# skyhehe123/SA-SSD

Measured on NVIDIA H100. Metric: KITTI frames/sec (~20k pts, car_cfg voxel grid), higher is better.
Workload: dtype f32

## Files before the change

sa-ssd_b200/csrc/spconv_split.cu:

```cuda
#include "tc_common.cuh"

namespace sps {

using namespace tc;

constexpr int BKC = 64;
constexpr int PROD_WARPS = 8;
constexpr int THREADS3 = CONS_THREADS + PROD_WARPS * 32;
constexpr int W_PROD = CONS_THREADS / 32;
constexpr int CLUSTER = 2;
constexpr int SPLIT_TILES_MAX = 74;

template <int BN>
struct Cfg3 {
    static constexpr int B_TILE_BYTES = BN * 128;
    static constexpr int STAGE_BYTES = 2 * A_TILE_BYTES + 2 * B_TILE_BYTES;
    static constexpr int STAGES = 4;
    static constexpr int NBR_TILE_BYTES = BM * 27 * 4;
    static constexpr int SMEM_BYTES = STAGES * STAGE_BYTES + 2 * NBR_TILE_BYTES + 1024 + 512 + 256;
};

__device__ __forceinline__ void cp_async16(uint32_t dst, const void* src, uint32_t src_bytes) {
    asm volatile("cp.async.cg.shared.global [%0], [%1], 16, %2;" ::"r"(dst), "l"(src), "r"(src_bytes) : "memory");
}
__device__ __forceinline__ void st_shared_zero16(uint32_t dst) {
    asm volatile("st.shared.v4.b32 [%0], {%1, %1, %1, %1};" ::"r"(dst), "r"(0u) : "memory");
}
__device__ __forceinline__ void cp_async_arrive_noinc(uint32_t bar) {
    asm volatile("cp.async.mbarrier.arrive.noinc.shared::cta.b64 [%0];" ::"r"(bar) : "memory");
}
__device__ __forceinline__ void mbar_arrive_remote(uint32_t bar, uint32_t rank) {
    asm volatile(
        "{\n\t"
        ".reg .b32 ra;\n\t"
        "mapa.shared::cluster.u32 ra, %0, %1;\n\t"
        "mbarrier.arrive.release.cluster.shared::cluster.b64 _, [ra];\n\t"
        "}\n" ::"r"(bar), "r"(rank) : "memory");
}
__device__ __forceinline__ void mbar_wait_cluster(uint32_t bar, uint32_t parity) {
    asm volatile(
        "{\n\t"
        ".reg .pred p;\n\t"
        "WAITC_LOOP:\n\t"
        "mbarrier.try_wait.parity.acquire.cluster.shared::cta.b64 p, [%0], %1;\n\t"
        "@p bra.uni WAITC_DONE;\n\t"
        "bra.uni WAITC_LOOP;\n\t"
        "WAITC_DONE:\n\t"
        "}\n" ::"r"(bar), "r"(parity) : "memory");
}

struct Args {
    const __half* in;
    size_t in_plane;
    const void* wpack;
    const float* scale;
    const float* shift;
    const int* nbr;
    const int* tile_mask;
    const int* d_rows;
    __half* out_split;
    size_t out_plane;
    float* out_f32;
    float* scratch;
    int* counters;
    int cin, cout, taps, rows_cap, relu, out_ch, out_f32_stride;
};

struct ChunkSet {
    uint32_t mask;
    __device__ __forceinline__ ChunkSet(uint32_t tap_mask, int tpg, int nchunks, int part, int nparts) {
        uint32_t act = tap_mask;
        if (tpg > 1) {
            const uint32_t group = (1u << tpg) - 1u;
            act = 0u;
            for (int g = 0; g < nchunks; ++g)
                if ((tap_mask >> (g * tpg)) & group) act |= 1u << g;
        }
        if (nparts == 1) { mask = act; return; }
        uint32_t m = 0u, rest = act;
        for (int j = 0; rest; ++j) {
            const uint32_t low = rest & (0u - rest);
            if ((j & 1) == part) m |= low;
            rest ^= low;
        }
        mask = m;
    }
};

template <int TABLE, int BN>
__global__ void __cluster_dims__(CLUSTER, 1, 1) __launch_bounds__(THREADS3, 1) spconv_split_kernel(const Args p) {
    using C = Cfg3<BN>;
    extern __shared__ uint8_t smem_raw[];
    const uint32_t base = (smem_u32(smem_raw) + 1023u) & ~1023u;
    uint8_t* base_ptr = smem_raw + (base - smem_u32(smem_raw));
    const uint32_t nbr_base = base + C::STAGES * C::STAGE_BYTES;
    const int* nbr_smem = (const int*)(base_ptr + C::STAGES * C::STAGE_BYTES);
    const uint32_t bar_base = nbr_base + 2 * C::NBR_TILE_BYTES;
    auto full_a = [&](int s, int w) { return bar_base + 512u + 8u * (s * PROD_WARPS + w); };
    auto full_b = [&](int s) { return bar_base + 8u * (C::STAGES + s); };
    auto empty = [&](int s) { return bar_base + 8u * (3 * C::STAGES + s); };
    auto nbr_full = [&](int b) { return bar_base + 8u * (4 * C::STAGES + 4 + b); };
    auto nbr_empty = [&](int b) { return bar_base + 8u * (4 * C::STAGES + 6 + b); };
    const uint32_t peer_done = bar_base + 8u * (4 * C::STAGES + 8);

    pdl_launch_dependents();
    const int warp = __shfl_sync(0xffffffffu, (int)(threadIdx.x >> 5), 0), lane = threadIdx.x & 31;
    const int cin = p.cin;
    const int ppt = cin >> 3;
    const int tpg = (BKC % cin == 0) ? BKC / cin : 1;
    const int nchunks = (p.taps + tpg - 1) / tpg;
    const bool nbr_tiles = TABLE && p.taps <= 27;
    const uint32_t all_taps = p.taps >= 32 ? 0xffffffffu : ((1u << p.taps) - 1u);

    if (threadIdx.x == 0) {
        for (int s = 0; s < C::STAGES; ++s) {
            for (int w = 0; w < PROD_WARPS; ++w) mbar_init(full_a(s, w), 32);
            mbar_init(full_b(s), 1);
            mbar_init(empty(s), 2);
        }
        for (int b = 0; b < 2; ++b) { mbar_init(nbr_full(b), 1); mbar_init(nbr_empty(b), PROD_WARPS); }
        mbar_init(peer_done, 128);
        fence_barrier_init();
    }
    __syncthreads();
    cluster_sync_all();
    pdl_wait();
    const int M = p.d_rows ? min(__ldg(p.d_rows), p.rows_cap) : p.rows_cap;
    const int ntiles = (M + BM - 1) / BM;
    const uint32_t crank = cluster_ctarank();
    const int G = (int)gridDim.x;
    const int R = ntiles / G, rem = ntiles - R * G;
    const bool tail_split = TABLE && p.scratch && nchunks > 1 && R == 0 && rem > 0 && 2 * rem <= G &&
                            rem <= SPLIT_TILES_MAX;
    const int n_items = R + ((tail_split ? (int)(blockIdx.x >> 1) < rem : (int)blockIdx.x < rem) ? 1 : 0);
    struct Item { int tile, part, nparts; };
    auto item_at = [&](int i) {
        Item it;
        if (i < R) { it.tile = (int)blockIdx.x + i * G; it.part = 0; it.nparts = 1; }
        else if (tail_split) { it.tile = R * G + (int)(blockIdx.x >> 1); it.part = (int)crank; it.nparts = 2; }
        else { it.tile = R * G + (int)blockIdx.x; it.part = 0; it.nparts = 1; }
        return it;
    };
    auto chunks_of = [&](const Item& it) {
        uint32_t tm = all_taps;
        if (TABLE && p.tile_mask) {
            tm = (uint32_t)__ldg(&p.tile_mask[it.tile]) & all_taps;
            if (!tm) tm = 1u;
        }
        return ChunkSet(tm, tpg, nchunks, it.part, it.nparts).mask;
    };
    auto rot_of = [&](int tile) { return (int)(((unsigned)tile * 11u) % (unsigned)nchunks); };

    if (warp >= W_PROD) {
        const int pw = warp - W_PROD;
        const bool loader = pw == 0 && lane == 0;
        const int piece = lane & 7, oct = lane >> 3;
        const int tl = piece / ppt, pc8 = (piece - tl * ppt) * 8;
        uint32_t offs[4];
        int rowt[4];
#pragma unroll
        for (int j = 0; j < 4; ++j) {
            const int r = pw * 16 + j * 4 + oct;
            offs[j] = (uint32_t)(r >> 3) * 1024u + (uint32_t)(r & 7) * 128u + (((uint32_t)piece ^ (uint32_t)(r & 7)) << 4);
            rowt[j] = r * p.taps;
        }
        const __half* in_hi = p.in + pc8;
        const __half* in_lo = in_hi + p.in_plane;
        int stage = 0;
        uint32_t phase = 0;
        int nb = 0;
        uint32_t nb_phase = 0;
        int ld_nb = 0;
        uint32_t ld_nb_phase = 0;
        auto load_nbr = [&](int tile) {
            const int rows_here = min(BM, p.rows_cap - tile * BM);
            const uint32_t bytes = (uint32_t)(rows_here * p.taps * 4) & ~15u;
            mbar_wait(nbr_empty(ld_nb), ld_nb_phase ^ 1u);
            mbar_expect_tx(nbr_full(ld_nb), bytes);
            if (bytes) bulk_g2s(nbr_base + ld_nb * C::NBR_TILE_BYTES, p.nbr + (size_t)tile * BM * p.taps, bytes, nbr_full(ld_nb));
            if (++ld_nb == 2) { ld_nb = 0; ld_nb_phase ^= 1u; }
        };
        if (loader && nbr_tiles && n_items > 0) load_nbr(item_at(0).tile);
        for (int ii = 0; ii < n_items; ++ii) {
            const Item item = item_at(ii);
            const int tile = item.tile;
            const int rows_here = min(BM, p.rows_cap - tile * BM);
            const int rows_copied = nbr_tiles ? ((rows_here * p.taps * 4) & ~15) / (p.taps * 4) : 0;
            const int* ntile = nbr_smem + nb * (C::NBR_TILE_BYTES / 4);
            const uint32_t cmask = chunks_of(item);
            const int m0 = tile * BM + pw * 16 + oct;
            if (nbr_tiles) {
                if (lane == 0) mbar_wait(nbr_full(nb), nb_phase);
                __syncwarp();
            }
            const int rot = rot_of(tile);
            auto chunk_at = [&](int gi) { return gi + rot < nchunks ? gi + rot : gi + rot - nchunks; };
            auto next_active = [&](int gi) {
                for (++gi; gi < nchunks; ++gi)
                    if ((cmask >> chunk_at(gi)) & 1u) break;
                return gi;
            };
            auto load_srcs = [&](int g, int (&dst)[4]) {
                const int t = g * tpg + tl;
                const bool tap_ok = tl < tpg && t < p.taps;
#pragma unroll
                for (int j = 0; j < 4; ++j) {
                    const int m = m0 + 4 * j;
                    dst[j] = -1;
                    if (tap_ok && m < M)
                        dst[j] = TABLE ? ((nbr_tiles && pw * 16 + j * 4 + oct < rows_copied) ? ntile[rowt[j] + t]
                                                                                          : __ldg(&p.nbr[(size_t)m * p.taps + t])) : m;
                }
            };
            int gi = next_active(-1);
            int srcs[4] = {-1, -1, -1, -1};
            if (gi < nchunks) load_srcs(chunk_at(gi), srcs);
            while (gi < nchunks) {
                const int gi_next = next_active(gi);
                if (lane == 0) {
                    mbar_wait(empty(stage), phase ^ 1u);
                    if (loader) {
                        const uint32_t dst = base + stage * C::STAGE_BYTES + 2 * A_TILE_BYTES;
                        const uint8_t* src = (const uint8_t*)p.wpack + (size_t)chunk_at(gi) * (2 * C::B_TILE_BYTES);
                        mbar_expect_tx(full_b(stage), 2 * C::B_TILE_BYTES);
                        bulk_g2s(dst, src, 2 * C::B_TILE_BYTES, full_b(stage));
                    }
                }
                __syncwarp();
                int nxt[4] = {-1, -1, -1, -1};
                if (gi_next < nchunks) load_srcs(chunk_at(gi_next), nxt);
                const uint32_t a_hi = base + stage * C::STAGE_BYTES, a_lo = a_hi + A_TILE_BYTES;
#pragma unroll
                for (int j = 0; j < 4; ++j) {
                    const uint32_t nbytes = srcs[j] >= 0 ? 16u : 0u;
                    const uint32_t eo = (uint32_t)(srcs[j] < 0 ? 0 : srcs[j]) * (uint32_t)cin;
                    cp_async16(a_hi + offs[j], in_hi + eo, nbytes);
                    cp_async16(a_lo + offs[j], in_lo + eo, nbytes);
                }
                cp_async_arrive_noinc(full_a(stage, pw));
                if (++stage == C::STAGES) { stage = 0; phase ^= 1u; }
#pragma unroll
                for (int j = 0; j < 4; ++j) srcs[j] = nxt[j];
                gi = gi_next;
            }
            if (nbr_tiles) {
                __syncwarp();
                if (lane == 0) mbar_arrive(nbr_empty(nb));
                if (++nb == 2) { nb = 0; nb_phase ^= 1u; }
            }
            if (loader && nbr_tiles && ii + 1 < n_items) load_nbr(item_at(ii + 1).tile);
        }
    } else {
        const int wg = threadIdx.x >> 7, t = threadIdx.x & 127;
        float big[BN / 2], small[BN / 2];
        int stage = 0;
        uint32_t phase = 0;
        int executed = 0, tiles_done = 0;
        for (int ii = 0; ii < n_items; ++ii) {
            const Item item = item_at(ii);
            const int tile = item.tile, part = item.part;
            const bool split = item.nparts == 2;
            const uint32_t cmask = chunks_of(item);
#pragma unroll
            for (int i = 0; i < BN / 2; ++i) { big[i] = 0.f; small[i] = 0.f; }
            const int rot = rot_of(tile);
            int prev = -1;
            for (int ci = 0; ci < nchunks; ++ci) {
                const int ch = ci + rot < nchunks ? ci + rot : ci + rot - nchunks;
                if (!((cmask >> ch) & 1u)) continue;
#pragma unroll 1
                for (int w = 0; w < PROD_WARPS; ++w) mbar_wait(full_a(stage, w), phase);
                fence_proxy_async();
                mbar_wait(full_b(stage), phase);
                const uint32_t ah = base + stage * C::STAGE_BYTES + (uint32_t)wg * (A_TILE_BYTES / 2);
                const uint32_t bh = base + stage * C::STAGE_BYTES + 2 * A_TILE_BYTES;
                wgmma_fence();
                mma_chunk_x3<1, BN>(big, small, ah, ah + A_TILE_BYTES, bh, bh + C::B_TILE_BYTES);
                wgmma_commit();
                wgmma_wait<1>();
                if (prev >= 0 && t == 0) mbar_arrive(empty(prev));
                prev = stage;
                ++executed;
                if (++stage == C::STAGES) { stage = 0; phase ^= 1u; }
            }
            wgmma_wait<0>();
            fence_regs<BN / 2>(big);
            fence_regs<BN / 2>(small);
            if (prev >= 0 && t == 0) mbar_arrive(empty(prev));
            if (part == 0) ++tiles_done;
            const bool giver = split && wg != part;
            const int rl0 = wg * 64 + (t >> 5) * 16 + ((t & 31) >> 2);
            float* prow = split ? p.scratch + (size_t)(tile - R * G) * BM * BN : nullptr;
            if (split && !giver) {
                mbar_wait_cluster(peer_done, 0u);
            }
#pragma unroll
            for (int j = 0; j < BN / 8; ++j) {
                const int n = 8 * j + 2 * (t & 3);
                const float scl0 = (p.scale && n < p.cout) ? __ldg(&p.scale[n]) : 1.f;
                const float scl1 = (p.scale && n + 1 < p.cout) ? __ldg(&p.scale[n + 1]) : 1.f;
                const float shl0 = (p.shift && n < p.cout) ? __ldg(&p.shift[n]) : 0.f;
                const float shl1 = (p.shift && n + 1 < p.cout) ? __ldg(&p.shift[n + 1]) : 0.f;
#pragma unroll
                for (int i = 0; i < 2; ++i) {
                    const int rl = rl0 + 8 * i, m = tile * BM + rl;
                    float a0 = __fadd_rn(big[4 * j + 2 * i], small[4 * j + 2 * i] * (1.f / kF16LoScale));
                    float a1 = __fadd_rn(big[4 * j + 2 * i + 1], small[4 * j + 2 * i + 1] * (1.f / kF16LoScale));
                    float2* q = split ? (float2*)(prow + (size_t)rl * BN + n) : nullptr;
                    if (giver) {
                        *q = make_float2(a0, a1);
                        continue;
                    }
                    if (split) {
                        const float2 pq = __ldcg(q);
                        a0 = __fadd_rn(a0, pq.x);
                        a1 = __fadd_rn(a1, pq.y);
                    }
                    float o0 = fmaf(a0, scl0, shl0), o1 = fmaf(a1, scl1, shl1);
                    if (p.relu) { o0 = fmaxf(o0, 0.f); o1 = fmaxf(o1, 0.f); }
                    if (m < M) {
                        if (p.out_f32 && n < p.out_f32_stride)
                            *(float2*)(p.out_f32 + (size_t)m * p.out_f32_stride + n) = make_float2(o0, o1);
                        if (p.out_split && 8 * j < p.out_ch) {
                            uint32_t h, l;
                            split_f16x2(o0, o1, h, l);
                            __half* ohi = p.out_split + (size_t)m * p.out_ch + n;
                            *(uint32_t*)ohi = h;
                            *(uint32_t*)(ohi + p.out_plane) = l;
                        }
                    }
                }
            }
            if (giver) mbar_arrive_remote(peer_done, (uint32_t)(part ^ 1));
        }
        if (p.counters && threadIdx.x == 0 && executed) {
            atomicAdd(&p.counters[0], executed);
            atomicAdd(&p.counters[1], tiles_done);
        }
    }

    __syncthreads();
    cluster_sync_all();
}

template <int TABLE, int BN>
static int launch3(const Args& a, cudaStream_t stream) {
    using C = Cfg3<BN>;
    auto kern = spconv_split_kernel<TABLE, BN>;
    static int max_ctas = 0;
    if (!max_ctas) {
        if (cudaFuncSetAttribute(kern, cudaFuncAttributeMaxDynamicSharedMemorySize, C::SMEM_BYTES) != cudaSuccess)
            return SASSD_ERR_LAUNCH;
        cudaLaunchConfig_t cfg = {};
        cfg.gridDim = dim3(CLUSTER * sassd_div_up(sassd_num_sms(), CLUSTER)); cfg.blockDim = dim3(THREADS3);
        cfg.dynamicSmemBytes = C::SMEM_BYTES;
        int clusters = 0;
        if (cudaOccupancyMaxActiveClusters(&clusters, kern, &cfg) != cudaSuccess || clusters < 1) {
            cudaGetLastError();
            clusters = sassd_num_sms() / (2 * CLUSTER);
        }
        max_ctas = CLUSTER * (clusters < SPLIT_TILES_MAX ? clusters : SPLIT_TILES_MAX);
    }
    int grid = CLUSTER * sassd_div_up(a.rows_cap, BM);
    if (grid > max_ctas) grid = max_ctas;
    if (launch_pdl(kern, dim3(grid), dim3(THREADS3), C::SMEM_BYTES, stream, a) != cudaSuccess) return SASSD_ERR_LAUNCH;
    return sassd_check_launch();
}

template <int TABLE>
static int dispatch3(const Args& a, cudaStream_t s) {
    if (a.cout <= 16) return launch3<TABLE, 16>(a, s);
    if (a.cout <= 32) return launch3<TABLE, 32>(a, s);
    if (a.cout <= 64) return launch3<TABLE, 64>(a, s);
    return SASSD_ERR_UNSUPPORTED;
}

}

__global__ void spconv_pack_kernel(const float* __restrict__ w, int taps, int cin, int cs, int cout, int bn, int tpg,
                                   int nchunks, __half* __restrict__ out) {
    const long long per_chunk = 2LL * bn * 64;
    const long long total = (long long)nchunks * per_chunk;
    for (long long i = blockIdx.x * (long long)blockDim.x + threadIdx.x; i < total; i += (long long)gridDim.x * blockDim.x) {
        const int g = (int)(i / per_chunk);
        long long rem = i % per_chunk;
        const int part = (int)(rem / (bn * 64));
        rem %= (bn * 64);
        const int n = (int)(rem / 64), pos = (int)(rem % 64);
        const int kk = (((pos >> 3) ^ (n & 7)) << 3) + (pos & 7);
        const int tl = kk / cs, ch = kk % cs, t = g * tpg + tl;
        float v = 0.f;
        if (tl < tpg && t < taps && ch < cin && n < cout) v = w[((size_t)t * cin + ch) * cout + n];
        float hi, lo;
        tc::split_f16(v, hi, lo);
        out[i] = __float2half_rn(part == 0 ? hi : lo);
    }
}

static int spconv_bn(int cout) { return cout <= 16 ? 16 : (cout <= 32 ? 32 : 64); }
static int spconv_tpg(int cs) { return (64 % cs == 0) ? 64 / cs : 1; }

extern "C" size_t sassd_spconv_pack_bytes(int taps, int cin_stored, int cout) {
    if (taps < 1 || cin_stored < 8 || (cin_stored & 7) || cin_stored > 64 || cout < 1 || cout > 64) return 0;
    const int tpg = spconv_tpg(cin_stored);
    return (size_t)((taps + tpg - 1) / tpg) * 2 * spconv_bn(cout) * 128;
}

extern "C" int sassd_spconv_pack(const float* weight, int taps, int cin, int cin_stored, int cout, void* packed,
                                 sassd_stream_t stream_) {
    if (!weight || !packed || cin < 1 || cin > cin_stored || !sassd_spconv_pack_bytes(taps, cin_stored, cout))
        return SASSD_ERR_ARG;
    const int tpg = spconv_tpg(cin_stored), nchunks = (taps + tpg - 1) / tpg, bn = spconv_bn(cout);
    spconv_pack_kernel<<<sassd_grid((long long)nchunks * 2 * bn * 64, 256), 256, 0, (cudaStream_t)stream_>>>(
        weight, taps, cin, cin_stored, cout, bn, tpg, nchunks, (__half*)packed);
    return sassd_check_launch();
}

extern "C" size_t sassd_spconv_workspace_bytes(void) {
    return (size_t)sps::SPLIT_TILES_MAX * sps::BM * 64 * sizeof(float);
}

extern "C" int sassd_spconv_f16x3(const sassd_spconv_desc* d, const void* in_split, const void* wpack,
                                  const float* scale, const float* shift, const int32_t* nbr,
                                  const int32_t* tile_mask, const int32_t* d_rows, void* out_split, float* out_f32,
                                  void* ws, size_t ws_bytes, int32_t* counters, sassd_stream_t stream_) {
    if (!d || !in_split || !wpack || (!out_split && !out_f32)) return SASSD_ERR_ARG;
    if (d->cin < 8 || (d->cin & 7) || d->cin > 64 || d->cout < 1 || d->cout > 64 || d->taps < 1 || d->rows_cap < 0)
        return SASSD_ERR_ARG;
    if (d->taps > 1 && !nbr) return SASSD_ERR_ARG;
    if (tile_mask && d->taps > 27) return SASSD_ERR_ARG;
    if (out_split && ((d->out_ch & 7) || d->out_ch < d->cout)) return SASSD_ERR_ARG;
    if (out_f32 && (d->out_f32_stride & 3)) return SASSD_ERR_ARG;
    if (ws && ws_bytes < sassd_spconv_workspace_bytes()) return SASSD_ERR_WORKSPACE;
    if (d->rows_cap == 0) return SASSD_OK;
    sps::Args a;
    a.in = (const __half*)in_split; a.in_plane = (size_t)d->in_rows_cap * d->cin;
    a.wpack = wpack; a.scale = scale; a.shift = shift; a.nbr = nbr; a.tile_mask = tile_mask; a.d_rows = d_rows;
    a.out_split = (__half*)out_split; a.out_plane = (size_t)d->rows_cap * d->out_ch; a.out_f32 = out_f32;
    a.scratch = (float*)ws; a.counters = counters;
    a.cin = d->cin; a.cout = d->cout; a.taps = d->taps; a.rows_cap = d->rows_cap; a.relu = d->relu;
    a.out_ch = d->out_ch; a.out_f32_stride = d->out_f32_stride;
    return d->taps > 1 ? sps::dispatch3<1>(a, (cudaStream_t)stream_) : sps::dispatch3<0>(a, (cudaStream_t)stream_);
}

__global__ void features_to_split_kernel(const float* __restrict__ feat, const int* __restrict__ d_rows, int rows_cap,
                                         int cin, int cs, __half* __restrict__ out) {
    const int rows = d_rows ? min(*d_rows, rows_cap) : rows_cap;
    const long long total = (long long)rows * cs;
    const size_t plane = (size_t)rows_cap * cs;
    for (long long i = blockIdx.x * (long long)blockDim.x + threadIdx.x; i < total; i += (long long)gridDim.x * blockDim.x) {
        const int r = (int)(i / cs), c = (int)(i % cs);
        float hi = 0.f, lo = 0.f;
        if (c < cin) tc::split_f16(feat[(size_t)r * cin + c], hi, lo);
        out[i] = __float2half_rn(hi);
        out[i + plane] = __float2half_rn(lo);
    }
}

extern "C" int sassd_features_to_split(const float* feat, const int32_t* d_rows, int rows_cap, int cin, int cs,
                                       void* out_split, sassd_stream_t stream_) {
    if (!feat || !out_split || cin < 1 || cs < cin || (cs & 7)) return SASSD_ERR_ARG;
    if (rows_cap <= 0) return SASSD_OK;
    features_to_split_kernel<<<sassd_grid((long long)rows_cap * cs, 256), 256, 0, (cudaStream_t)stream_>>>(
        feat, d_rows, rows_cap, cin, cs, (__half*)out_split);
    return sassd_check_launch();
}

__global__ void split_rows_to_bev_kernel(const uint4* __restrict__ feat, size_t in_plane16, const int4* __restrict__ coors,
                                         const int* __restrict__ d_rows, int rows_cap, int C8, int D, int H, int W,
                                         size_t out_plane16, uint4* __restrict__ bev, int* __restrict__ tile_dist) {
    const int rows = min(*d_rows, rows_cap);
    const long long total = (long long)rows * C8;
    for (long long i = blockIdx.x * (long long)blockDim.x + threadIdx.x; i < total; i += (long long)gridDim.x * blockDim.x) {
        const int r = (int)(i / C8), q = (int)(i % C8);
        const int4 c = __ldg(&coors[r]);
        const size_t o = (((size_t)c.x * H + c.z) * W + c.w) * (size_t)(D * C8) + (size_t)c.y * C8 + q;
        bev[o] = __ldg(&feat[i]);
        bev[o + out_plane16] = __ldg(&feat[i + in_plane16]);
        if (tile_dist && q == 0) sassd_mark_conv2d_tiles(tile_dist, c.x, c.z, c.w, H, W);
    }
}

extern "C" int sassd_split_rows_to_bev(const void* feat_split, const int32_t* coors, const int32_t* d_rows, int rows_cap,
                                       int C, int D, int H, int W, int batch, void* bev_split, int32_t* tile_dist,
                                       sassd_stream_t stream_) {
    if (!feat_split || !coors || !d_rows || !bev_split || (C & 7) || batch < 1) return SASSD_ERR_ARG;
    if (rows_cap <= 0) return SASSD_OK;
    const size_t in_plane16 = (size_t)rows_cap * C / 8, out_plane16 = (size_t)batch * H * W * D * C / 8;
    split_rows_to_bev_kernel<<<sassd_grid((long long)rows_cap * (C / 8), 256), 256, 0, (cudaStream_t)stream_>>>(
        (const uint4*)feat_split, in_plane16, (const int4*)coors, d_rows, rows_cap, C / 8, D, H, W, out_plane16,
        (uint4*)bev_split, tile_dist);
    return sassd_check_launch();
}
```

sa-ssd_b200/ops.py:

```python
import collections
import ctypes
import os
import math

import numpy as np
import torch

from . import lib as _lib
from .lib import Conv2dDesc, SpconvDesc
from .lib import (GCONV_CONV2D, GCONV_ROWS, GCONV_TABLE, PREC_F16X3, PREC_FP32, PREC_TF32X3, GConvDesc, VoxelParams,
                  check)

NMS_CAP = 4096
DEFAULT_PRECISION = PREC_F16X3


def _L():
    return _lib.load()


def _stream():
    return ctypes.c_void_p(torch.cuda.current_stream().cuda_stream)


def _ptr(t):
    if t is None:
        return ctypes.c_void_p(0)
    assert t.is_cuda and t.is_contiguous(), "sassd ops need contiguous CUDA tensors"
    return ctypes.c_void_p(t.data_ptr())


def require_cuda():
    if not torch.cuda.is_available():
        raise _lib.SassdError("sassd_b200 needs a CUDA device (sm_90a); there is no CPU fallback")


def next_pow2(n):
    return 1 << max(1, int(math.ceil(math.log2(max(2, n)))))


_KERNELS = {"sassd_voxelize": 4, "sassd_voxel_mean": 1, "sassd_frustum_crop": 1,"sassd_anchor_mask": 4, "sassd_hash_build": 1,
            "sassd_rulebook_subm": 1, "sassd_rulebook_conv_outputs": 2, "sassd_rulebook_conv_outputs_hash": 2, "sassd_rulebook_conv_nbr": 1,
            "sassd_rulebook_pairs": 1, "sassd_gconv": 1, "sassd_gconv_pack": 1, "sassd_spconv_pack": 1, "sassd_rotate_overlap_eval": 1, "sassd_conv2d_f16x3": 1, "sassd_conv2d_f16x3_occ": 1, "sassd_conv2d_f16x3_occ_bg": 1, "sassd_spconv_f16x3": 1, "sassd_features_to_split": 1, "sassd_split_rows_to_bev": 1, "sassd_sparse_to_bev_split": 1, "sassd_sparse_to_bev": 1, "sassd_decode_select": 2,
            "sassd_pswarp": 1, "sassd_rescore_nms": 3, "sassd_kitti_format": 1, "sassd_three_nn": 1, "sassd_point_aux_head": 1, "sassd_nms_mask": 1, "sassd_nms_sorted": 2,
            "sassd_boxes_iou_bev": 1, "sassd_points_in_boxes": 2, "sassd_assign_rpn": 3, "sassd_assign_pswarp": 3,
            "sassd_rpn_loss": 2, "sassd_pswarp_loss": 2, "sassd_aux_loss": 2}
LAUNCHES = 0
PROFILE = None


def _call(name, label, *args):
    global LAUNCHES
    LAUNCHES += _KERNELS[name]
    fn = getattr(_L(), name)
    if PROFILE is None:
        check(fn(*args), name)
        return
    e0 = torch.cuda.Event(enable_timing=True)
    e1 = torch.cuda.Event(enable_timing=True)
    e0.record()
    check(fn(*args), name)
    e1.record()
    PROFILE.append((name, label, e0, e1))


class Workspace:

    def __init__(self):
        self._bufs = {}

    def get(self, key, nbytes, device):
        buf = self._bufs.get(key)
        if buf is None or buf.numel() < nbytes or buf.device != device:
            buf = torch.empty(max(int(nbytes), 256), dtype=torch.uint8, device=device)
            self._bufs[key] = buf
        return buf


_WS = Workspace()


def make_voxel_params(voxel_size, pc_range, max_points, max_voxels):
    vs = np.asarray(voxel_size, np.float32)
    rg = np.asarray(pc_range, np.float32)
    grid = np.round((rg[3:] - rg[:3]) / vs).astype(np.int64)
    p = VoxelParams()
    for j in range(3):
        p.voxel_size[j] = float(vs[j]); p.range_min[j] = float(rg[j]); p.grid[j] = int(grid[j])
    p.max_points = int(max_points); p.max_voxels = int(max_voxels)
    return p, grid


def voxelize(points, pt_off, batch, params, rows_cap, slots_per_frame, status, want_mean=True, ws=None):
    dev = points.device
    n_cap = points.shape[0]
    voxels = torch.empty((rows_cap, params.max_points, 4), dtype=torch.float32, device=dev)
    coors = torch.empty((rows_cap, 4), dtype=torch.int32, device=dev)
    num = torch.empty((rows_cap,), dtype=torch.int32, device=dev)
    mean = torch.empty((rows_cap, 4), dtype=torch.float32, device=dev) if want_mean else None
    frame_rows = torch.empty((batch + 1,), dtype=torch.int32, device=dev)
    nbytes = _L().sassd_voxelize_workspace_bytes(n_cap, batch, slots_per_frame)
    w = (ws or _WS).get("voxelize", nbytes, dev)
    _call("sassd_voxelize", None, _ptr(points), _ptr(pt_off), n_cap, batch, ctypes.byref(params), slots_per_frame,
                              _ptr(voxels), _ptr(coors), _ptr(num), _ptr(mean), rows_cap, _ptr(frame_rows),
                              _ptr(status), _ptr(w), w.numel(), _stream())
    return voxels, coors, num, mean, frame_rows


def frustum_crop(points, pt_off, batch, planes, ws=None):
    dev = points.device
    n_cap = points.shape[0]
    assert planes.dtype == torch.float64 and tuple(planes.shape) == (batch, 6, 4), "planes must be float64 [batch,6,4]"
    out = torch.empty_like(points)
    off = torch.empty((batch + 1,), dtype=torch.int32, device=dev)
    nbytes = _L().sassd_frustum_crop_workspace_bytes(n_cap, batch)
    w = (ws or _WS).get("frustum", nbytes, dev)
    _call("sassd_frustum_crop", None, _ptr(points), _ptr(pt_off), n_cap, batch, _ptr(planes), _ptr(out), _ptr(off),
          _ptr(w), w.numel(), _stream())
    return out, off


def voxel_mean(voxels, num_points, d_rows=None):
    rows, maxp = voxels.shape[0], voxels.shape[1]
    mean = torch.empty((rows, 4), dtype=torch.float32, device=voxels.device)
    _call("sassd_voxel_mean", None, _ptr(voxels), _ptr(num_points), _ptr(d_rows), rows, maxp, _ptr(mean), _stream())
    return mean


def anchor_mask(coors, d_rows, batch, H, W, rects, threshold=1, ws=None):
    dev = coors.device
    na = rects.shape[0]
    mask = torch.empty((batch, na), dtype=torch.uint8, device=dev)
    nbytes = _L().sassd_anchor_mask_workspace_bytes(batch, H, W)
    w = (ws or _WS).get("amask", nbytes, dev)
    _call("sassd_anchor_mask", None, _ptr(coors), _ptr(d_rows), coors.shape[0], batch, H, W, _ptr(rects), na,
                                 int(threshold), _ptr(mask), _ptr(w), w.numel(), _stream())
    return mask


class HashIndex:
    def __init__(self, rows_cap, device):
        self.slots = next_pow2(2 * max(rows_cap, 1))
        self.keys = torch.empty((self.slots,), dtype=torch.int32, device=device)
        self.vals = torch.empty((self.slots,), dtype=torch.int32, device=device)


def hash_build(index, coors, d_rows, batch, shape, status):
    D, H, W = shape
    _call("sassd_hash_build", None, _ptr(coors), _ptr(d_rows), coors.shape[0], batch, D, H, W, _ptr(index.keys),
                                _ptr(index.vals), index.slots, _ptr(status), _stream())
    return index


def _tile_mask_buffer(rows_cap, device):
    n = (rows_cap + _lib.SPCONV_TILE_ROWS - 1) // _lib.SPCONV_TILE_ROWS
    return torch.empty((max(n, 1),), dtype=torch.int32, device=device)


def rulebook_subm(coors, d_rows, shape, index, nbr=None):
    D, H, W = shape
    rows_cap = coors.shape[0]
    if nbr is None:
        nbr = torch.empty((rows_cap, 27), dtype=torch.int32, device=coors.device)
    tmask = _tile_mask_buffer(rows_cap, coors.device)
    _call("sassd_rulebook_subm", None, _ptr(coors), _ptr(d_rows), rows_cap, D, H, W, _ptr(index.keys), _ptr(index.vals),
                                   index.slots, _ptr(nbr), _ptr(tmask), _stream())
    return nbr, tmask


def conv_out_shape(shape):
    return [(s + 2 - 3) // 2 + 1 for s in shape]


def rulebook_conv_outputs(coors_in, d_rows_in, batch, shape, rows_cap_out, status, ws=None, ws_key="rbconv",
                          index_out=None):
    dev = coors_in.device
    D, H, W = shape
    Do, Ho, Wo = conv_out_shape(shape)
    coors_out = torch.empty((rows_cap_out, 4), dtype=torch.int32, device=dev)
    d_rows_out = torch.empty((1,), dtype=torch.int32, device=dev)
    nbytes = _L().sassd_rulebook_conv_workspace_bytes(batch, Do, Ho, Wo)
    w = (ws or _WS).get(ws_key, nbytes, dev)
    if index_out is None:
        _call("sassd_rulebook_conv_outputs", None, _ptr(coors_in), _ptr(d_rows_in), coors_in.shape[0], batch, D, H, W,
              _ptr(coors_out), _ptr(d_rows_out), rows_cap_out, _ptr(status), _ptr(w), w.numel(), _stream())
    else:
        _call("sassd_rulebook_conv_outputs_hash", None, _ptr(coors_in), _ptr(d_rows_in), coors_in.shape[0], batch, D, H, W,
              _ptr(coors_out), _ptr(d_rows_out), rows_cap_out, _ptr(index_out.keys), _ptr(index_out.vals),
              index_out.slots, _ptr(status), _ptr(w), w.numel(), _stream())
    return coors_out, d_rows_out, [Do, Ho, Wo]


def rulebook_conv_nbr(coors_out, d_rows_out, shape_in, index_in):
    D, H, W = shape_in
    rows_cap_out = coors_out.shape[0]
    nbr = torch.empty((rows_cap_out, 27), dtype=torch.int32, device=coors_out.device)
    tmask = _tile_mask_buffer(rows_cap_out, coors_out.device)
    _call("sassd_rulebook_conv_nbr", None, _ptr(coors_out), _ptr(d_rows_out), rows_cap_out, D, H, W, _ptr(index_in.keys),
          _ptr(index_in.vals), index_in.slots, _ptr(nbr), _ptr(tmask), _stream())
    return nbr, tmask


def rulebook_conv(coors_in, d_rows_in, batch, shape, index_in, rows_cap_out, status, ws=None, ws_key="rbconv",
                  index_out=None):
    coors_out, d_rows_out, so = rulebook_conv_outputs(coors_in, d_rows_in, batch, shape, rows_cap_out, status, ws, ws_key,
                                                      index_out)
    nbr, tmask = rulebook_conv_nbr(coors_out, d_rows_out, shape, index_in)
    return coors_out, d_rows_out, nbr, so, tmask


def rulebook_pairs(nbr, d_rows):
    rows_cap = nbr.shape[0]
    pairs = torch.empty((2, 27, rows_cap), dtype=torch.int32, device=nbr.device)
    num = torch.empty((27,), dtype=torch.int32, device=nbr.device)
    _call("sassd_rulebook_pairs", None, _ptr(nbr), _ptr(d_rows), rows_cap, _ptr(pairs), _ptr(num), _stream())
    return pairs, num


_TC_PACKS = {}


def pack_tc(weight, precision):
    taps, cin, cout = weight.shape
    nbytes = _L().sassd_gconv_pack_bytes(taps, cin, cout, precision)
    packed = torch.empty((nbytes,), dtype=torch.uint8, device=weight.device)
    _call("sassd_gconv_pack", None, _ptr(weight), taps, cin, cout, precision, _ptr(packed), _stream())
    return packed
# ... 278 lines not shown
TILE_OCCUPANCY = os.environ.get("SASSD_TMA_OCC", "1") != "0"
CONV2D_TILE_ORDER = 0
CONV2D_COUNTERS = None
_TILE_FAR = 1 << 20


def _tile_dist(batch, H, W, device):
    if not TILE_OCCUPANCY:
        return None
    th, tw = _lib.CONV2D_TILE_H, _lib.CONV2D_TILE_W
    return torch.full((batch * ((H + th - 1) // th) * ((W + tw - 1) // tw),), _TILE_FAR, dtype=torch.int32, device=device)


def tile_skipping_valid(H, W, reach):
    th, tw = _lib.CONV2D_TILE_H, _lib.CONV2D_TILE_W
    if reach > _lib.TILE_DIST_MAX:
        return False
    last_h = H - (H - 1) // th * th
    last_w = W - (W - 1) // tw * tw
    return min(last_h, last_w, th, tw) >= reach - 1


_CONV_CONSTS = {}


def conv_constant(x_const, cin, weight, scale, shift, relu, cout):
    key = (weight.data_ptr(), weight._version, None if scale is None else (scale.data_ptr(), scale._version),
           None if shift is None else (shift.data_ptr(), shift._version), bool(relu), cout, cin,
           None if x_const is None else x_const.data_ptr())
    ent = _CONV_CONSTS.get(key)
    if ent is None:
        if len(_CONV_CONSTS) >= 256:
            _CONV_CONSTS.pop(next(iter(_CONV_CONSTS)))
        h, w = 3 * _lib.CONV2D_TILE_H, 3 * _lib.CONV2D_TILE_W
        m = torch.zeros((1, h, w, cin), dtype=torch.float32, device=weight.device)
        if x_const is not None:
            m += x_const[:cin].view(1, 1, 1, cin)
        _, f = conv2d_split(SplitMap.from_float(m), weight, scale, shift, relu, cout, out_split=False, out_f32=True)
        ent = (f[0, h // 2, w // 2, :cout].clone().contiguous(), weight, scale, shift, x_const)
        _CONV_CONSTS[key] = ent
    return ent[0]


_BACKGROUNDS = collections.OrderedDict()
BACKGROUND_CACHE_BYTES = 4 << 30
BACKGROUND_PINS = None


def conv_background(x, weight, scale, shift, relu, cout, out_split, out_f32):
    B, H, W, cin = x.shape
    src = x.background
    if src is None and x.reach > 0:
        return None
    key = (weight.data_ptr(), weight._version, None if scale is None else (scale.data_ptr(), scale._version),
           None if shift is None else (shift.data_ptr(), shift._version), bool(relu), cout, cin, x.planes.shape[-1], H, W,
           None if src is None else src.planes.data_ptr(), bool(out_split), bool(out_f32))
    ent = _BACKGROUNDS.get(key)
    if ent is None:
        if src is None:
            src_in = SplitMap(torch.zeros((2, 1, H, W, x.planes.shape[-1]), dtype=torch.float16, device=x.device), cin)
        else:
            src_in = src
        bg = conv2d_split(src_in, weight, scale, shift, relu, cout, out_split=out_split, out_f32=out_f32)
        nbytes = sum(t.numel() * t.element_size() for t in (bg[0] and bg[0].planes, bg[1]) if t is not None)
        ent = (bg, nbytes, weight, scale, shift, src)
        _BACKGROUNDS[key] = ent
        while len(_BACKGROUNDS) > 1 and sum(e[1] for e in _BACKGROUNDS.values()) > BACKGROUND_CACHE_BYTES:
            _BACKGROUNDS.popitem(last=False)
    else:
        _BACKGROUNDS.move_to_end(key)
    if BACKGROUND_PINS is not None:
        BACKGROUND_PINS.append(ent[0])
    return ent[0]


def sparse_to_bev_split(feat, coors, d_rows, C, D, H, W, batch):
    planes = torch.zeros((2, batch, H, W, D * C), dtype=torch.float16, device=feat.device)
    dist = _tile_dist(batch, H, W, feat.device)
    _call("sassd_sparse_to_bev_split", None, _ptr(feat), _ptr(coors), _ptr(d_rows), feat.shape[0], C, D, H, W, batch,
          _ptr(planes), _ptr(dist), _stream())
    return SplitMap(planes, D * C, dist)


def conv2d_split(x, weight, scale, shift, relu, cout, out_split=True, out_f32=False):
    B, H, W, cin = x.shape
    taps = weight.shape[0]
    wp = tc_pack_cached(weight, PREC_F16X3)
    d = Conv2dDesc()
    d.batch, d.H, d.W, d.cin, d.cin_stored = B, H, W, cin, x.planes.shape[-1]
    d.cout, d.taps, d.relu = cout, taps, 1 if relu else 0
    d.tile_order = CONV2D_TILE_ORDER
    d.n_split = 0
    osp = of = None
    if out_split:
        cs = (cout + 63) // 64 * 64
        alloc = torch.empty if cs == cout else torch.zeros
        osp = alloc((2, B, H, W, cs), dtype=torch.float16, device=x.device)
        d.out_split_ch = cs
    if out_f32:
        stride = (cout + 3) // 4 * 4
        of = torch.empty((B, H, W, stride), dtype=torch.float32, device=x.device)
        d.out_f32_stride = stride
    label = "conv2d_tma[taps=%d %d->%d]" % (taps, cin, cout)
    dist = x.tile_dist if TILE_OCCUPANCY else None
    reach, cvec, bg_sp, bg_f = 0, None, None, None
    if dist is not None:
        reach = x.reach + (1 if taps == 9 else 0)
        if not tile_skipping_valid(H, W, reach):
            dist = None
    if dist is not None:
        cvec = conv_constant(x.const, cin, weight, scale, shift, relu, cout)
        bg = conv_background(x, weight, scale, shift, relu, cout, out_split, out_f32)
        if bg is not None:
            bg_sp, bg_f = bg
    _call("sassd_conv2d_f16x3_occ_bg", label, ctypes.byref(d), _ptr(x.planes), _ptr(wp), _ptr(scale), _ptr(shift),
          _ptr(of), _ptr(osp), _ptr(dist), reach, _ptr(cvec), _ptr(bg_sp.planes if bg_sp is not None else None),
          _ptr(bg_f), _ptr(CONV2D_COUNTERS.get(label) if CONV2D_COUNTERS is not None else None), _stream())
    return (SplitMap(osp, cout, dist, reach, cvec, bg_sp) if osp is not None else None), of


def features_to_split(feat, d_rows=None):
    cap, C = feat.shape
    cs = (C + 7) // 8 * 8
    out = torch.empty((2, cap, cs), dtype=torch.float16, device=feat.device)
    _call("sassd_features_to_split", None, _ptr(feat), _ptr(d_rows), cap, C, cs, _ptr(out), _stream())
    return out


def split_rows_float(planes, channels):
    return (planes[0].float() + planes[1].float() * (1.0 / 2048.0))[:, :channels].contiguous()


SPCONV_COUNTERS = None
SPCONV_TAP_SKIP = os.environ.get("SASSD_SPS_SKIP", "1") != "0"
SPCONV_TAP_SPLIT = os.environ.get("SASSD_SPS_SPLIT", "1") != "0"


def spconv_split(planes, weight, scale, shift, relu, cout, rows_cap, nbr=None, d_rows=None, want_f32=False,
                 tile_mask=None, ws=None):
    taps = weight.shape[0]
    wp = spconv_pack_cached(weight, planes.shape[2])
    d = SpconvDesc()
    d.cin, d.cout, d.taps = planes.shape[2], cout, taps
    d.rows_cap, d.in_rows_cap, d.relu = rows_cap, planes.shape[1], 1 if relu else 0
    d.out_ch = (cout + 7) // 8 * 8
    out = torch.empty((2, rows_cap, d.out_ch), dtype=torch.float16, device=planes.device)
    of = None
    if want_f32:
        d.out_f32_stride = (cout + 3) // 4 * 4
        of = torch.empty((rows_cap, d.out_f32_stride), dtype=torch.float32, device=planes.device)
    label = "spconv_split[taps=%d %d->%d]" % (taps, weight.shape[1], cout)
    w = None
    if SPCONV_TAP_SPLIT and taps > 1:
        w = (ws or _WS).get("spconv_split", _L().sassd_spconv_workspace_bytes(), planes.device)
    _call("sassd_spconv_f16x3", label, ctypes.byref(d), _ptr(planes), _ptr(wp), _ptr(scale), _ptr(shift), _ptr(nbr),
          _ptr(tile_mask if SPCONV_TAP_SKIP else None), _ptr(d_rows), _ptr(out), _ptr(of), _ptr(w),
          0 if w is None else w.numel(), _ptr(SPCONV_COUNTERS), _stream())
    return out, of


def split_rows_to_bev(planes, coors, d_rows, C, D, H, W, batch):
    bev = torch.zeros((2, batch, H, W, D * C), dtype=torch.float16, device=planes.device)
    dist = _tile_dist(batch, H, W, planes.device)
    _call("sassd_split_rows_to_bev", None, _ptr(planes), _ptr(coors), _ptr(d_rows), planes.shape[1], C, D, H, W, batch,
          _ptr(bev), _ptr(dist), _stream())
    return SplitMap(bev, D * C, dist)
```

Baseline: 774.1.

## Replace cluster tail-split with balanced chunk dealing across CTAs

Drops the 2-CTA cluster tail split and adds a work-dealing scheme. Each CTA prefix-scans the active tap chunks per tile and takes a contiguous range of chunks across tiles, so load balances over up to 148 CTAs when the longest tile clearly dominates. Partial sums go to a global parts buffer, and the last arriving CTA, found with an acq_rel atomic counter, reduces them and runs the epilogue. This removes cluster launch limits and idle CTAs on skewed tiles, at the cost of a per-CTA scan, global partial traffic, and a zeroed arrivals workspace.

```diff
diff --git a/sa-ssd_b200/csrc/spconv_split.cu b/sa-ssd_b200/csrc/spconv_split.cu
--- a/sa-ssd_b200/csrc/spconv_split.cu
+++ b/sa-ssd_b200/csrc/spconv_split.cu
@@ -8,8 +8,8 @@
 constexpr int PROD_WARPS = 8;
 constexpr int THREADS3 = CONS_THREADS + PROD_WARPS * 32;
 constexpr int W_PROD = CONS_THREADS / 32;
-constexpr int CLUSTER = 2;
-constexpr int SPLIT_TILES_MAX = 74;
+constexpr int MAX_CTAS = 148;
+constexpr int DEAL_MIN_GAIN = 14;
 
 template <int BN>
 struct Cfg3 {
@@ -17,7 +17,9 @@
     static constexpr int STAGE_BYTES = 2 * A_TILE_BYTES + 2 * B_TILE_BYTES;
     static constexpr int STAGES = 4;
     static constexpr int NBR_TILE_BYTES = BM * 27 * 4;
-    static constexpr int SMEM_BYTES = STAGES * STAGE_BYTES + 2 * NBR_TILE_BYTES + 1024 + 512 + 256;
+    static constexpr int BAR_BYTES = 768;
+    static constexpr int DEAL_INTS = MAX_CTAS + 1 + 33 + 2 + 1;
+    static constexpr int SMEM_BYTES = STAGES * STAGE_BYTES + 2 * NBR_TILE_BYTES + 1024 + BAR_BYTES + DEAL_INTS * 4;
 };
 
 __device__ __forceinline__ void cp_async16(uint32_t dst, const void* src, uint32_t src_bytes) {
@@ -29,24 +31,13 @@
 __device__ __forceinline__ void cp_async_arrive_noinc(uint32_t bar) {
     asm volatile("cp.async.mbarrier.arrive.noinc.shared::cta.b64 [%0];" ::"r"(bar) : "memory");
 }
-__device__ __forceinline__ void mbar_arrive_remote(uint32_t bar, uint32_t rank) {
-    asm volatile(
-        "{\n\t"
-        ".reg .b32 ra;\n\t"
-        "mapa.shared::cluster.u32 ra, %0, %1;\n\t"
-        "mbarrier.arrive.release.cluster.shared::cluster.b64 _, [ra];\n\t"
-        "}\n" ::"r"(bar), "r"(rank) : "memory");
-}
-__device__ __forceinline__ void mbar_wait_cluster(uint32_t bar, uint32_t parity) {
-    asm volatile(
-        "{\n\t"
-        ".reg .pred p;\n\t"
-        "WAITC_LOOP:\n\t"
-        "mbarrier.try_wait.parity.acquire.cluster.shared::cta.b64 p, [%0], %1;\n\t"
-        "@p bra.uni WAITC_DONE;\n\t"
-        "bra.uni WAITC_LOOP;\n\t"
-        "WAITC_DONE:\n\t"
-        "}\n" ::"r"(bar), "r"(parity) : "memory");
+__device__ __forceinline__ void warpgroup_sync(int id) {
+    asm volatile("bar.sync %0, 128;" ::"r"(id) : "memory");
+}
+__device__ __forceinline__ int atomic_add_acq_rel(int* p, int v) {
+    int old;
+    asm volatile("atom.acq_rel.gpu.global.add.s32 %0, [%1], %2;" : "=r"(old) : "l"(p), "r"(v) : "memory");
+    return old;
 }
 
 struct Args {
@@ -61,34 +52,35 @@
     __half* out_split;
     size_t out_plane;
     float* out_f32;
-    float* scratch;
+    float* parts;
+    int* arrivals;
     int* counters;
     int cin, cout, taps, rows_cap, relu, out_ch, out_f32_stride;
 };
 
-struct ChunkSet {
-    uint32_t mask;
-    __device__ __forceinline__ ChunkSet(uint32_t tap_mask, int tpg, int nchunks, int part, int nparts) {
-        uint32_t act = tap_mask;
-        if (tpg > 1) {
-            const uint32_t group = (1u << tpg) - 1u;
-            act = 0u;
-            for (int g = 0; g < nchunks; ++g)
-                if ((tap_mask >> (g * tpg)) & group) act |= 1u << g;
-        }
-        if (nparts == 1) { mask = act; return; }
-        uint32_t m = 0u, rest = act;
-        for (int j = 0; rest; ++j) {
-            const uint32_t low = rest & (0u - rest);
-            if ((j & 1) == part) m |= low;
-            rest ^= low;
-        }
-        mask = m;
-    }
-};
+__device__ __forceinline__ uint32_t active_chunks(uint32_t tap_mask, int tpg, int nchunks) {
+    if (tpg == 1) return tap_mask;
+    const uint32_t group = (1u << tpg) - 1u;
+    uint32_t act = 0u;
+    for (int g = 0; g < nchunks; ++g)
+        if ((tap_mask >> (g * tpg)) & group) act |= 1u << g;
+    return act;
+}
+
+__device__ __forceinline__ uint32_t chunk_range(uint32_t act, int rot, int nchunks, int lo, int hi) {
+    uint32_t m = 0u;
+    for (int gi = 0, r = 0; gi < nchunks; ++gi) {
+        const int g = gi + rot < nchunks ? gi + rot : gi + rot - nchunks;
+        if ((act >> g) & 1u) {
+            if (r >= lo && r < hi) m |= 1u << g;
+            ++r;
+        }
+    }
+    return m;
+}
 
 template <int TABLE, int BN>
-__global__ void __cluster_dims__(CLUSTER, 1, 1) __launch_bounds__(THREADS3, 1) spconv_split_kernel(const Args p) {
+__global__ void __launch_bounds__(THREADS3, 1) spconv_split_kernel(const Args p) {
     using C = Cfg3<BN>;
     extern __shared__ uint8_t smem_raw[];
     const uint32_t base = (smem_u32(smem_raw) + 1023u) & ~1023u;
@@ -101,7 +93,10 @@
     auto empty = [&](int s) { return bar_base + 8u * (3 * C::STAGES + s); };
     auto nbr_full = [&](int b) { return bar_base + 8u * (4 * C::STAGES + 4 + b); };
     auto nbr_empty = [&](int b) { return bar_base + 8u * (4 * C::STAGES + 6 + b); };
-    const uint32_t peer_done = bar_base + 8u * (4 * C::STAGES + 8);
+    int* deal_pre = (int*)(base_ptr + C::STAGES * C::STAGE_BYTES + 2 * C::NBR_TILE_BYTES + C::BAR_BYTES);
+    int* scan_smem = deal_pre + MAX_CTAS + 1;
+    int* last_flag = scan_smem + 33;
+    int* longest = last_flag + 2;
 
     pdl_launch_dependents();
     const int warp = __shfl_sync(0xffffffffu, (int)(threadIdx.x >> 5), 0), lane = threadIdx.x & 31;
@@ -119,37 +114,71 @@
             mbar_init(empty(s), 2);
         }
         for (int b = 0; b < 2; ++b) { mbar_init(nbr_full(b), 1); mbar_init(nbr_empty(b), PROD_WARPS); }
-        mbar_init(peer_done, 128);
         fence_barrier_init();
-    }
-    __syncthreads();
-    cluster_sync_all();
+        *longest = 0;
+    }
     pdl_wait();
     const int M = p.d_rows ? min(__ldg(p.d_rows), p.rows_cap) : p.rows_cap;
     const int ntiles = (M + BM - 1) / BM;
-    const uint32_t crank = cluster_ctarank();
     const int G = (int)gridDim.x;
-    const int R = ntiles / G, rem = ntiles - R * G;
-    const bool tail_split = TABLE && p.scratch && nchunks > 1 && R == 0 && rem > 0 && 2 * rem <= G &&
-                            rem <= SPLIT_TILES_MAX;
-    const int n_items = R + ((tail_split ? (int)(blockIdx.x >> 1) < rem : (int)blockIdx.x < rem) ? 1 : 0);
-    struct Item { int tile, part, nparts; };
+    auto active_of = [&](int tile) {
+        uint32_t tm = all_taps;
+        if (TABLE && p.tile_mask) {
+            tm = (uint32_t)__ldg(&p.tile_mask[tile]) & all_taps;
+            if (!tm) tm = 1u;
+        }
+        return active_chunks(tm, tpg, nchunks);
+    };
+    auto rot_of = [&](int tile) { return (int)(((unsigned)tile * 11u) % (unsigned)nchunks); };
+    const bool may_deal = TABLE && p.arrivals && ntiles > 0 && ntiles <= G;
+    if (may_deal) {
+        const int t = (int)threadIdx.x, cnt = t < ntiles ? __popc(active_of(t)) : 0;
+        int total;
+        const int pre = sassd_block_exscan(cnt, scan_smem, &total);
+        if (t < ntiles) deal_pre[t] = pre;
+        if (t == 0) deal_pre[ntiles] = total;
+        const int wmax = __reduce_max_sync(0xffffffffu, cnt);
+        if (lane == 0) atomicMax(longest, wmax);
+    }
+    __syncthreads();
+    const bool deal = may_deal && *longest - (deal_pre[ntiles] + G - 1) / G >= DEAL_MIN_GAIN;
+    const int S = deal ? deal_pre[ntiles] : 1, D = min(G, S);
+    const bool dealt = deal && (int)blockIdx.x < D;
+    const int s0 = dealt ? (int)blockIdx.x * S / D : 0;
+    const int s1 = dealt ? ((int)blockIdx.x + 1) * S / D : 0;
+    auto tile_of = [&](int k) {
+        int lo = 0, hi = ntiles - 1;
+        while (lo < hi) {
+            const int mid = (lo + hi + 1) >> 1;
+            if (deal_pre[mid] <= k) lo = mid; else hi = mid - 1;
+        }
+        return lo;
+    };
+    auto owner_of = [&](int k) { return ((k + 1) * D - 1) / S; };
+    const int t_first = s1 > s0 ? tile_of(s0) : 0;
+    const int R = ntiles / G;
+    const int n_items = deal ? (s1 > s0 ? tile_of(s1 - 1) - t_first + 1 : 0)
+                             : R + ((int)blockIdx.x < ntiles - R * G ? 1 : 0);
+    struct Item { int tile, lo, hi; };
     auto item_at = [&](int i) {
         Item it;
-        if (i < R) { it.tile = (int)blockIdx.x + i * G; it.part = 0; it.nparts = 1; }
-        else if (tail_split) { it.tile = R * G + (int)(blockIdx.x >> 1); it.part = (int)crank; it.nparts = 2; }
-        else { it.tile = R * G + (int)blockIdx.x; it.part = 0; it.nparts = 1; }
+        if (deal) {
+            it.tile = t_first + i;
+            const int b = deal_pre[it.tile];
+            it.lo = max(s0 - b, 0);
+            it.hi = min(s1, deal_pre[it.tile + 1]) - b;
+        } else {
+            it.tile = (int)blockIdx.x + i * G;
+            it.lo = 0;
+            it.hi = 32;
+        }
         return it;
     };
     auto chunks_of = [&](const Item& it) {
-        uint32_t tm = all_taps;
-        if (TABLE && p.tile_mask) {
-            tm = (uint32_t)__ldg(&p.tile_mask[it.tile]) & all_taps;
-            if (!tm) tm = 1u;
-        }
-        return ChunkSet(tm, tpg, nchunks, it.part, it.nparts).mask;
+        const uint32_t act = active_of(it.tile);
+        if (it.lo == 0 && it.hi >= __popc(act)) return act;
+        return chunk_range(act, rot_of(it.tile), nchunks, it.lo, it.hi);
     };
-    auto rot_of = [&](int tile) { return (int)(((unsigned)tile * 11u) % (unsigned)nchunks); };
 
     if (warp >= W_PROD) {
         const int pw = warp - W_PROD;
@@ -258,8 +287,7 @@
         int executed = 0, tiles_done = 0;
         for (int ii = 0; ii < n_items; ++ii) {
             const Item item = item_at(ii);
-            const int tile = item.tile, part = item.part;
-            const bool split = item.nparts == 2;
+            const int tile = item.tile;
             const uint32_t cmask = chunks_of(item);
 #pragma unroll
             for (int i = 0; i < BN / 2; ++i) { big[i] = 0.f; small[i] = 0.f; }
@@ -287,13 +315,42 @@
             fence_regs<BN / 2>(big);
             fence_regs<BN / 2>(small);
             if (prev >= 0 && t == 0) mbar_arrive(empty(prev));
-            if (part == 0) ++tiles_done;
-            const bool giver = split && wg != part;
+#pragma unroll
+            for (int i = 0; i < BN / 2; ++i) big[i] = __fadd_rn(big[i], small[i] * (1.f / kF16LoScale));
+            if (deal && (item.lo > 0 || item.hi < deal_pre[tile + 1] - deal_pre[tile])) {
+                const int b = deal_pre[tile], e = deal_pre[tile + 1];
+                const int first = owner_of(b), nparts = owner_of(e - 1) - first + 1;
+                const int part = (int)blockIdx.x - first;
+                auto slot = [&](int j) {
+                    const int c = first + j, s = 2 * c + ((j == 0 && c * S / D < b) ? 1 : 0);
+                    return (float2*)(p.parts + ((size_t)s * BM + wg * 64) * BN) + t;
+                };
+                float2* mine = slot(part);
+#pragma unroll
+                for (int k = 0; k < BN / 4; ++k) __stcg(mine + 128 * k, make_float2(big[2 * k], big[2 * k + 1]));
+                warpgroup_sync(1 + wg);
+                if (t == 0) {
+                    int* arrived = p.arrivals + 2 * tile + wg;
+                    const bool last = atomic_add_acq_rel(arrived, 1) == nparts - 1;
+                    if (last) *arrived = 0;
+                    last_flag[wg] = last;
+                }
+                warpgroup_sync(1 + wg);
+                if (!last_flag[wg]) continue;
+                for (int j = 0; j < nparts; ++j) {
+                    const float2* q = slot(j);
+#pragma unroll
+                    for (int k = 0; k < BN / 4; ++k) {
+                        const float2 v = j == part ? make_float2(big[2 * k], big[2 * k + 1]) : __ldcg(q + 128 * k);
+                        small[2 * k] = j == 0 ? v.x : __fadd_rn(small[2 * k], v.x);
+                        small[2 * k + 1] = j == 0 ? v.y : __fadd_rn(small[2 * k + 1], v.y);
+                    }
+                }
+#pragma unroll
+                for (int i = 0; i < BN / 2; ++i) big[i] = small[i];
+            }
+            ++tiles_done;
             const int rl0 = wg * 64 + (t >> 5) * 16 + ((t & 31) >> 2);
-            float* prow = split ? p.scratch + (size_t)(tile - R * G) * BM * BN : nullptr;
-            if (split && !giver) {
-                mbar_wait_cluster(peer_done, 0u);
-            }
 #pragma unroll
             for (int j = 0; j < BN / 8; ++j) {
                 const int n = 8 * j + 2 * (t & 3);
@@ -303,20 +360,8 @@
                 const float shl1 = (p.shift && n + 1 < p.cout) ? __ldg(&p.shift[n + 1]) : 0.f;
 #pragma unroll
                 for (int i = 0; i < 2; ++i) {
-                    const int rl = rl0 + 8 * i, m = tile * BM + rl;
-                    float a0 = __fadd_rn(big[4 * j + 2 * i], small[4 * j + 2 * i] * (1.f / kF16LoScale));
-                    float a1 = __fadd_rn(big[4 * j + 2 * i + 1], small[4 * j + 2 * i + 1] * (1.f / kF16LoScale));
-                    float2* q = split ? (float2*)(prow + (size_t)rl * BN + n) : nullptr;
-                    if (giver) {
-                        *q = make_float2(a0, a1);
-                        continue;
-                    }
-                    if (split) {
-                        const float2 pq = __ldcg(q);
-                        a0 = __fadd_rn(a0, pq.x);
-                        a1 = __fadd_rn(a1, pq.y);
-                    }
-                    float o0 = fmaf(a0, scl0, shl0), o1 = fmaf(a1, scl1, shl1);
+                    const int m = tile * BM + rl0 + 8 * i;
+                    float o0 = fmaf(big[4 * j + 2 * i], scl0, shl0), o1 = fmaf(big[4 * j + 2 * i + 1], scl1, shl1);
                     if (p.relu) { o0 = fmaxf(o0, 0.f); o1 = fmaxf(o1, 0.f); }
                     if (m < M) {
                         if (p.out_f32 && n < p.out_f32_stride)
@@ -331,7 +376,6 @@
                     }
                 }
             }
-            if (giver) mbar_arrive_remote(peer_done, (uint32_t)(part ^ 1));
         }
         if (p.counters && threadIdx.x == 0 && executed) {
             atomicAdd(&p.counters[0], executed);
@@ -340,38 +384,28 @@
     }
 
     __syncthreads();
-    cluster_sync_all();
 }
 
 template <int TABLE, int BN>
-static int launch3(const Args& a, cudaStream_t stream) {
+static int launch3(const Args& a, int max_work, cudaStream_t stream) {
     using C = Cfg3<BN>;
     auto kern = spconv_split_kernel<TABLE, BN>;
-    static int max_ctas = 0;
-    if (!max_ctas) {
+    static bool smem_set = false;
+    if (!smem_set) {
         if (cudaFuncSetAttribute(kern, cudaFuncAttributeMaxDynamicSharedMemorySize, C::SMEM_BYTES) != cudaSuccess)
             return SASSD_ERR_LAUNCH;
-        cudaLaunchConfig_t cfg = {};
-        cfg.gridDim = dim3(CLUSTER * sassd_div_up(sassd_num_sms(), CLUSTER)); cfg.blockDim = dim3(THREADS3);
-        cfg.dynamicSmemBytes = C::SMEM_BYTES;
-        int clusters = 0;
-        if (cudaOccupancyMaxActiveClusters(&clusters, kern, &cfg) != cudaSuccess || clusters < 1) {
-            cudaGetLastError();
-            clusters = sassd_num_sms() / (2 * CLUSTER);
-        }
-        max_ctas = CLUSTER * (clusters < SPLIT_TILES_MAX ? clusters : SPLIT_TILES_MAX);
-    }
-    int grid = CLUSTER * sassd_div_up(a.rows_cap, BM);
-    if (grid > max_ctas) grid = max_ctas;
+        smem_set = true;
+    }
+    const int grid = min(max_work, min(sassd_num_sms(), MAX_CTAS));
     if (launch_pdl(kern, dim3(grid), dim3(THREADS3), C::SMEM_BYTES, stream, a) != cudaSuccess) return SASSD_ERR_LAUNCH;
     return sassd_check_launch();
 }
 
 template <int TABLE>
-static int dispatch3(const Args& a, cudaStream_t s) {
-    if (a.cout <= 16) return launch3<TABLE, 16>(a, s);
-    if (a.cout <= 32) return launch3<TABLE, 32>(a, s);
-    if (a.cout <= 64) return launch3<TABLE, 64>(a, s);
+static int dispatch3(const Args& a, int max_work, cudaStream_t s) {
+    if (a.cout <= 16) return launch3<TABLE, 16>(a, max_work, s);
+    if (a.cout <= 32) return launch3<TABLE, 32>(a, max_work, s);
+    if (a.cout <= 64) return launch3<TABLE, 64>(a, max_work, s);
     return SASSD_ERR_UNSUPPORTED;
 }
 
@@ -416,8 +450,10 @@
     return sassd_check_launch();
 }
 
+static size_t spconv_parts_bytes() { return (size_t)2 * sps::MAX_CTAS * sps::BM * 64 * sizeof(float); }
+
 extern "C" size_t sassd_spconv_workspace_bytes(void) {
-    return (size_t)sps::SPLIT_TILES_MAX * sps::BM * 64 * sizeof(float);
+    return spconv_parts_bytes() + (size_t)sps::MAX_CTAS * 2 * sizeof(int32_t);
 }
 
 extern "C" int sassd_spconv_f16x3(const sassd_spconv_desc* d, const void* in_split, const void* wpack,
@@ -437,10 +473,14 @@
     a.in = (const __half*)in_split; a.in_plane = (size_t)d->in_rows_cap * d->cin;
     a.wpack = wpack; a.scale = scale; a.shift = shift; a.nbr = nbr; a.tile_mask = tile_mask; a.d_rows = d_rows;
     a.out_split = (__half*)out_split; a.out_plane = (size_t)d->rows_cap * d->out_ch; a.out_f32 = out_f32;
-    a.scratch = (float*)ws; a.counters = counters;
+    a.parts = (float*)ws;
+    a.arrivals = ws ? (int*)((char*)ws + spconv_parts_bytes()) : nullptr;
+    a.counters = counters;
     a.cin = d->cin; a.cout = d->cout; a.taps = d->taps; a.rows_cap = d->rows_cap; a.relu = d->relu;
     a.out_ch = d->out_ch; a.out_f32_stride = d->out_f32_stride;
-    return d->taps > 1 ? sps::dispatch3<1>(a, (cudaStream_t)stream_) : sps::dispatch3<0>(a, (cudaStream_t)stream_);
+    const int tiles = sassd_div_up(d->rows_cap, sps::BM), tpg = spconv_tpg(d->cin);
+    if (d->taps == 1) return sps::dispatch3<0>(a, tiles, (cudaStream_t)stream_);
+    return sps::dispatch3<1>(a, ws ? tiles * ((d->taps + tpg - 1) / tpg) : tiles, (cudaStream_t)stream_);
 }
 
 __global__ void features_to_split_kernel(const float* __restrict__ feat, const int* __restrict__ d_rows, int rows_cap,
diff --git a/sa-ssd_b200/ops.py b/sa-ssd_b200/ops.py
--- a/sa-ssd_b200/ops.py
+++ b/sa-ssd_b200/ops.py
@@ -69,10 +69,10 @@
     def __init__(self):
         self._bufs = {}
 
-    def get(self, key, nbytes, device):
+    def get(self, key, nbytes, device, zeroed=False):
         buf = self._bufs.get(key)
         if buf is None or buf.numel() < nbytes or buf.device != device:
-            buf = torch.empty(max(int(nbytes), 256), dtype=torch.uint8, device=device)
+            buf = (torch.zeros if zeroed else torch.empty)(max(int(nbytes), 256), dtype=torch.uint8, device=device)
             self._bufs[key] = buf
         return buf
 
@@ -657,7 +657,7 @@
     label = "spconv_split[taps=%d %d->%d]" % (taps, weight.shape[1], cout)
     w = None
     if SPCONV_TAP_SPLIT and taps > 1:
-        w = (ws or _WS).get("spconv_split", _L().sassd_spconv_workspace_bytes(), planes.device)
+        w = (ws or _WS).get("spconv_split", _L().sassd_spconv_workspace_bytes(), planes.device, zeroed=True)
     _call("sassd_spconv_f16x3", label, ctypes.byref(d), _ptr(planes), _ptr(wp), _ptr(scale), _ptr(shift), _ptr(nbr),
           _ptr(tile_mask if SPCONV_TAP_SKIP else None), _ptr(d_rows), _ptr(out), _ptr(of), _ptr(w),
           0 if w is None else w.numel(), _ptr(SPCONV_COUNTERS), _stream())
```

After: 798.8 (median of 6 runs). +3.2%, better.
